# passcod/zarc

Hardware: AMD Instinct MI355X
Metric: uncompressed GiB/s (pack) at zstd -3 (higher is better)
Workload: dtype u8; 1 GPU; zarc pack 10000 x 1048576 B synthetic entries per GPU, zstd level 3, checksum on (BASELINE configs[1]); entries_per_gpu=10000, entries_total=10000, entry_bytes=1048576, level=3, kinds=text/records/lz/random round-robin

## Files before the change

### zarc_amd/csrc/zge_entropy.hip

```cpp
#include "zarc_device.h"
#include "zarc_kernels.h"
#include "zge_seq_join.h"

namespace {

#ifdef ZARC_HIPEMU
#define ZGE_CLOCK() 0ull
#else
#define ZGE_CLOCK() ((unsigned long long)__builtin_readcyclecounter())
#endif
#define ENT_PROF(i) do { if (prof && lane == 0) { const unsigned long long now_ = ZGE_CLOCK(); atomicAdd(prof + (i), now_ - tprev); tprev = now_; } } while (0)

constexpr int HUF_MAXBITS = 11;
constexpr uint32_t MIN_HUF_LITERALS = 64;

__constant__ const int16_t E_LL_DEFAULT[36] = {4, 3, 2, 2, 2, 2, 2, 2, 2, 2, 2, 2, 2, 1, 1, 1, 2, 2,
                                               2, 2, 2, 2, 2, 2, 2, 3, 2, 1, 1, 1, 1, 1, -1, -1, -1, -1};
__constant__ const int16_t E_ML_DEFAULT[53] = {1, 4, 3, 2, 2, 2, 2, 2, 2, 1, 1, 1, 1, 1, 1, 1, 1, 1,
                                               1, 1, 1, 1, 1, 1, 1, 1, 1, 1, 1, 1, 1, 1, 1, 1, 1, 1,
                                               1, 1, 1, 1, 1, 1, 1, 1, 1, 1, -1, -1, -1, -1, -1, -1, -1};
__constant__ const int16_t E_OF_DEFAULT[29] = {1, 1, 1, 1, 1, 1, 2, 2, 2, 1, 1, 1, 1, 1, 1,
                                               1, 1, 1, 1, 1, 1, 1, 1, 1, -1, -1, -1, -1, -1};
__device__ __forceinline__ uint32_t ll_code(uint32_t ll)
{
// ... 155 lines not shown
            rank++;
        }
    }
    zd::wave_sync();
    for (int i0 = 0; i0 < T; i0 += 64) {
        const int i = i0 + lane;
        const bool act = i < T;
        const uint32_t sym = act ? (uint32_t)cellsym[i] : 64u;
        uint64_t same = zd::ballot(act);
#pragma unroll
        for (int b = 0; b < 6; b++) { const uint64_t m = zd::ballot((sym >> b) & 1u); same &= ((sym >> b) & 1u) ? m : ~m; }
        const uint32_t below = (uint32_t)__popcll(same & ((1ull << lane) - 1)), all = (uint32_t)__popcll(same);
        int base = 0;
        if (act) base = t.dfs[sym];
        zd::wave_lds_order();
        if (act) {
            t.state_tab[base + (int)below] = (uint16_t)(T + i);
            if (below + 1 == all) t.dfs[sym] = base + (int)all;
        }
        zd::wave_lds_order();
    }
    zd::wave_sync();
    if (lane < nsym) {
        const int n = n_l, total = (int)start_all;
        if (n == 0) { t.dnb[lane] = ((al + 1) << 16) - T; t.dfs[lane] = 0; }
        else if (n == -1 || n == 1) { t.dnb[lane] = (al << 16) - T; t.dfs[lane] = total - 1; }
        else {
            const int max_bits_out = al - zd::hb32((uint32_t)(n - 1));
            t.dnb[lane] = (max_bits_out << 16) - (n << max_bits_out);
            t.dfs[lane] = total - n;
        }
    }
    t.al = al;
    zd::wave_sync();
}
__device__ __forceinline__ uint32_t fse_init_state(const FseCtab &t, int s)
{
    const int nb = (t.dnb[s] + (1 << 15)) >> 16;
    const int value = (nb << 16) - t.dnb[s];
    return t.state_tab[(value >> nb) + t.dfs[s]];
}
__device__ __forceinline__ uint32_t fse_step(const FseCtab &t, uint32_t state, int s, uint32_t *bits)
{
    const int nb = (int)((state + (uint32_t)t.dnb[s]) >> 16);
    *bits = (state & ((1u << nb) - 1)) | ((uint32_t)nb << 16);
    return t.state_tab[(int)(state >> nb) + t.dfs[s]];
}
__device__ uint32_t log2_fp8(uint32_t x)
{
    const int h = zd::hb32(x);
    const uint32_t frac = h >= 8 ? (x >> (h - 8)) - 256 : (x << (8 - h)) - 256;
    return (uint32_t)h * 256 + frac;
}
__device__ void fse_normalize(const uint32_t *count, int nsym, uint32_t total, int al, int16_t *norm)
{
    const int T = 1 << al;
    int sum = 0;
    for (int s = 0; s < nsym; s++) {
        if (count[s] == 0) { norm[s] = 0; continue; }
        uint64_t v = ((uint64_t)count[s] * (uint64_t)T + total / 2) / total;
        if (v < 1) v = 1;
        norm[s] = (int16_t)v;
        sum += (int)v;
    }
    while (sum != T) {
        int best = -1;
        for (int s = 0; s < nsym; s++) if (norm[s] > 0 && (best < 0 || norm[s] > norm[best])) best = s;
        if (sum > T) {
            int take = sum - T;
            const int room = norm[best] - 1;
            if (take > room) take = room;
            if (take <= 0) break;
            norm[best] = (int16_t)(norm[best] - take);
            sum -= take;
        } else {
            norm[best] = (int16_t)(norm[best] + (T - sum));
            sum = T;
        }
    }
}
__device__ uint32_t fse_write_desc(uint8_t *dst, uint32_t cap, const int16_t *norm, int nsym, int al)
{
    BitW b;
    b.init(dst, cap);
    int remaining = (1 << al) + 1, threshold = 1 << al, nb = al + 1, s = 0;
    b.add((uint32_t)(al - 5), 4);
    while (remaining > 1 && s < nsym) {
        const int count = norm[s++], max = 2 * threshold - 1 - remaining;
        int val = count + 1;
        remaining -= count < 0 ? -count : count;
        if (val >= threshold) val += max;
        if (val < max) b.add((uint32_t)val, nb - 1); else b.add((uint32_t)val, nb);
        if (count == 0) {
            int run = 0;
            while (s + run < nsym && norm[s + run] == 0) run++;
            s += run;
            while (run >= 3) { b.add(3, 2); run -= 3; }
            b.add((uint32_t)run, 2);
        }
        while (remaining < threshold) { nb--; threshold >>= 1; }
    }
    b.flush_partial();
    return b.overflow ? 0 : b.pos;
}
__device__ uint64_t dist_cost(const uint32_t *count, const int16_t *norm, int nsym, int al)
{
    uint64_t c = 0;
    for (int s = 0; s < nsym; s++) {
        if (!count[s]) continue;
        if (norm[s] == 0) return ~0ull;
        const uint32_t n = norm[s] < 0 ? 1u : (uint32_t)norm[s];
        c += (uint64_t)count[s] * ((uint32_t)al * 256 - log2_fp8(n));
    }
    return c;
}
__device__ void choose_table(EntLds &L, int which, const uint32_t *count, int maxsym, uint32_t nseq, const int16_t *def, int def_n,
                             int def_al, int max_al)
{
    int distinct = 0, last = 0;
    for (int s = 0; s <= maxsym; s++) if (count[s]) { distinct++; last = s; }
    int16_t *norm = L.s.norm[which];
    L.ctrl[X_COST_L + which] = 0;
    if (distinct == 1) { L.ctrl[X_MODE_L + which] = 1; L.ctrl[X_RLE_L + which] = last; L.ctrl[X_DL_L + which] = 0; return; }
    uint64_t cost_def = ~0ull;
    if (last < def_n) {
        for (int s = 0; s < def_n; s++) norm[s] = def[s];
        cost_def = dist_cost(count, norm, def_n, def_al);
    }
    int al = zd::hb32(nseq > 1 ? nseq - 1 : 1) - 2;
    if (al > max_al) al = max_al;
    if (al < 5) al = 5;
    while ((1 << al) < distinct) al++;
    const int nsym = last + 1;
    fse_normalize(count, nsym, nseq, al, norm);
    const uint32_t dl = fse_write_desc(L.s.desc[which], 80, norm, nsym, al);
    const uint64_t cost_dyn = dl ? dist_cost(count, norm, nsym, al) + (uint64_t)dl * 8 * 256 : ~0ull;
    if (cost_def <= cost_dyn) {
        for (int s = 0; s < def_n; s++) norm[s] = def[s];
        L.ctrl[X_MODE_L + which] = 0; L.ctrl[X_NSYM_L + which] = def_n; L.ctrl[X_AL_L + which] = def_al; L.ctrl[X_DL_L + which] = 0;
        L.ctrl[X_COST_L + which] = (int)(uint32_t)cost_def;
    } else {
        L.ctrl[X_MODE_L + which] = 2; L.ctrl[X_NSYM_L + which] = nsym; L.ctrl[X_AL_L + which] = al; L.ctrl[X_DL_L + which] = (int)dl;
        L.ctrl[X_COST_L + which] = (int)(uint32_t)cost_dyn;
    }
}

__device__ int huf_build_lengths(EntLds &L, int lane)
{
    uint32_t present = 0;
    uint32_t *const keys = &L.h.w[256];
    {
        const uint64_t lt = (1ull << lane) - 1;
#pragma unroll
        for (int r = 0; r < 4; r++) {
            const int s = r * 64 + lane;
            const uint32_t c = L.h.count[s];
            L.h.len8[s] = 0;
            const uint64_t m = zd::ballot(c != 0);
            if (c) keys[present + (uint32_t)__popcll(m & lt)] = (c << 8) | (uint32_t)s;
            present += (uint32_t)__popcll(m);
        }
    }
    zd::wave_sync();
    for (uint32_t i = (uint32_t)lane; i < present; i += 64) {
        const uint32_t k = keys[i];
        uint32_t rank = 0;
        for (uint32_t t = 0; t < present; t++) rank += keys[t] < k ? 1u : 0u;
        L.h.order[rank] = (uint16_t)(k & 0xFF);
    }
    zd::wave_sync();
    const int n = (int)present;
    if (n < 2) { if (n == 1 && lane == 0) L.h.len8[L.h.order[0]] = 1; zd::wave_sync(); return n; }
    for (int i = lane; i < n; i += 64) L.h.w[i] = L.h.count[L.h.order[i]];
    zd::wave_sync();
    if (lane == 0) {
        int leaf = 0, inode = n, next = n;
        while (next < 2 * n - 1) {
            int a, b;
            if (leaf < n && (inode >= next || L.h.w[leaf] <= L.h.w[inode])) a = leaf++; else a = inode++;
            if (leaf < n && (inode >= next || L.h.w[leaf] <= L.h.w[inode])) b = leaf++; else b = inode++;
            L.h.w[next] = L.h.w[a] + L.h.w[b];
            L.h.parent[a] = (uint16_t)next;
            L.h.parent[b] = (uint16_t)next;
            next++;
        }
    }
    zd::wave_sync();
    int *const num = (int *)&L.h.w[0];
    {
        uint32_t dep[4];
#pragma unroll
        for (int r = 0; r < 4; r++) {
            const int i = r * 64 + lane;
            dep[r] = 0;
            if (i < n) { int j = i; uint32_t d = 0; while (j != 2 * n - 2) { j = L.h.parent[j]; d++; } dep[r] = d > 63 ? 63 : d; }
        }
        zd::wave_sync();
// ... 17 lines not shown
    {
        uint32_t cum[HUF_MAXBITS + 1];
        uint32_t c = 0;
#pragma unroll
        for (int k = 1; k <= HUF_MAXBITS; k++) { c += (uint32_t)num[k]; cum[k] = c; }
#pragma unroll
        for (int r = 0; r < 4; r++) {
            const int j = r * 64 + lane;
            if (j < n) {
                const uint32_t t = (uint32_t)(n - 1 - j);
                uint32_t k = 1;
#pragma unroll
                for (int q = 1; q < HUF_MAXBITS; q++) k += cum[q] <= t ? 1u : 0u;
                L.h.len8[L.h.order[j]] = (uint8_t)k;
            }
        }
    }
    zd::wave_sync();
    return n;
}

__device__ void huf_assign_codes(EntLds &L, int lane)
{
    uint32_t len[4], idx[4];
    uint32_t maxlen = 0, last = 0;
#pragma unroll
    for (int r = 0; r < 4; r++) { len[r] = L.h.len8[r * 64 + lane]; idx[r] = 0; if (len[r] > maxlen) maxlen = len[r]; if (len[r]) last = (uint32_t)(r * 64 + lane); }
    maxlen = zd::uniform(zd::wave_max(maxlen));
    last = zd::uniform(zd::wave_max(last));
    const uint64_t lt = (1ull << lane) - 1;
    uint32_t *const rank_start = &L.h.w[64];
    uint32_t pos = 0;
    for (uint32_t w = 1; w <= maxlen; w++) {
        const uint32_t lv = maxlen + 1 - w;
        uint32_t cnt = 0;
#pragma unroll
        for (int r = 0; r < 4; r++) {
            const uint64_t m = zd::ballot(len[r] == lv);
            if (len[r] == lv) idx[r] = cnt + (uint32_t)__popcll(m & lt);
            cnt += (uint32_t)__popcll(m);
        }
        if (lane == 0) rank_start[w] = pos;
        pos += cnt << (w - 1);
    }
    zd::wave_sync();
#pragma unroll
    for (int r = 0; r < 4; r++) {
        uint32_t code = 0;
        if (len[r]) { const uint32_t w = maxlen + 1 - len[r]; code = ((rank_start[w] >> (w - 1)) + idx[r]) | (len[r] << 11); }
        L.code[r * 64 + lane] = (uint16_t)code;
    }
    if (lane == 0) { L.ctrl[X_MAXBITS] = (int)maxlen; L.ctrl[X_NSYM_LAST] = (int)last; }
    zd::wave_sync();
}

__device__ uint32_t huf_write_desc(EntLds &L)
{
    const int n = L.ctrl[X_NSYM_LAST];
    if (n > 1) {
        int nsym = 0, distinct = 0, al = 6;
        uint32_t maxc = 0;
        for (int s = 0; s < 13; s++) if (L.h.cw[s]) { nsym = s + 1; distinct++; if (L.h.cw[s] > maxc) maxc = L.h.cw[s]; }
        if (distinct > 1 && maxc > 1) {
            { int lim = zd::hb32((uint32_t)(n - 1)) - 2; if (lim < al) al = lim; if (al < 5) al = 5; }
            while ((1 << al) < distinct) al++;
            fse_normalize(L.h.cw, nsym, (uint32_t)n, al, L.h.wnorm);
            const uint32_t hdr = fse_write_desc(L.h.tmp, 192, L.h.wnorm, nsym, al);
            if (hdr) {
                FseCtab ct = {L.h.st_w, L.h.dnb_w, L.h.dfs_w, 0};
                fse_build_ctab(ct, L.h.wnorm, nsym, al, L.cellsym);
                BitW b;
                b.init(L.h.tmp + hdr, 192 - hdr);
                uint32_t s1, s2, bits;
                int ip = n;
                if (n & 1) {
                    s1 = fse_init_state(ct, L.h.wt[--ip]);
                    s2 = fse_init_state(ct, L.h.wt[--ip]);
                    s1 = fse_step(ct, s1, L.h.wt[--ip], &bits); b.add(bits & 0xFFFF, (int)(bits >> 16));
                } else {
                    s2 = fse_init_state(ct, L.h.wt[--ip]);
                    s1 = fse_init_state(ct, L.h.wt[--ip]);
                }
                while (ip > 0) {
                    s2 = fse_step(ct, s2, L.h.wt[--ip], &bits); b.add(bits & 0xFFFF, (int)(bits >> 16));
                    s1 = fse_step(ct, s1, L.h.wt[--ip], &bits); b.add(bits & 0xFFFF, (int)(bits >> 16));
                }
                b.add(s2, al);
                b.add(s1, al);
                const uint32_t body = b.close();
                if (!b.overflow && hdr + body < 128 && (n > 128 || hdr + body < (uint32_t)(n + 1) / 2)) {
                    L.h.hdesc[0] = (uint8_t)(hdr + body);
                    for (uint32_t i = 0; i < hdr + body; i++) L.h.hdesc[1 + i] = L.h.tmp[i];
                    return 1 + hdr + body;
                }
            }
        }
    }
    if (n > 128) return 0;
    L.h.hdesc[0] = (uint8_t)(127 + n);
    for (int i = 0; i < n; i += 2) L.h.hdesc[1 + i / 2] = (uint8_t)((L.h.wt[i] << 4) | (i + 1 < n ? L.h.wt[i + 1] : 0));
    return (uint32_t)(1 + (n + 1) / 2);
}

struct WavePacker {
    uint32_t *stage;
    uint8_t *dst;
    uint32_t pos;
    uint32_t carry;
    uint32_t cap;
    bool overflow;
    __device__ void begin(uint32_t *st, uint8_t *d, uint32_t c, int lane)
    {
        stage = st; dst = d; pos = 0; carry = 0; cap = c; overflow = false;
        for (int i = lane; i < 224; i += 64) stage[i] = 0;
        zd::wave_sync();
    }
    __device__ void put(uint64_t lo, uint32_t hi, uint32_t nbits, int lane)
    {
        const uint32_t incl = zd::wave_scan_incl(nbits);
        const uint32_t total = zd::readlane(incl, 63);
        const uint32_t at = carry + incl - nbits;
        if (nbits) {
            const uint32_t w = at >> 5, sh = at & 31;
            const uint32_t v0 = (uint32_t)lo, v1 = (uint32_t)(lo >> 32), v2 = hi;
            const uint32_t o0 = v0 << sh;
            const uint32_t o1 = sh ? (v1 << sh) | (v0 >> (32 - sh)) : v1;
            const uint32_t o2 = sh ? (v2 << sh) | (v1 >> (32 - sh)) : v2;
            const uint32_t o3 = sh ? (v2 >> (32 - sh)) : 0u;
            if (o0) atomicOr(&stage[w], o0);
            if (o1) atomicOr(&stage[w + 1], o1);
            if (o2) atomicOr(&stage[w + 2], o2);
            if (o3) atomicOr(&stage[w + 3], o3);
        }
        zd::wave_sync();
        const uint32_t bits = carry + total, full = bits >> 3;
        const uint8_t *sb = (const uint8_t *)stage;
        if (pos + full + 1 > cap) overflow = true;
        if (!overflow) {
            const uint32_t fw = full >> 2;
            for (uint32_t i = (uint32_t)lane; i < fw; i += 64) { const uint32_t w = stage[i]; __builtin_memcpy(dst + pos + 4 * i, &w, 4); }
            if ((uint32_t)lane < (full & 3)) dst[pos + 4 * fw + (uint32_t)lane] = sb[4 * fw + (uint32_t)lane];
        }
        const uint32_t keep = (bits & 7) ? (uint32_t)sb[full] : 0u;
        zd::wave_sync();
        const uint32_t words = (bits + 31) / 32 + 1;
        for (uint32_t i = (uint32_t)lane; i < words; i += 64) stage[i] = i == 0 ? keep : 0u;
        zd::wave_sync();
        pos += full;
        carry = bits & 7;
    }
    __device__ uint32_t finish(int lane)
    {
        put(1, 0, lane == 0 ? 1u : 0u, lane);
        if (carry) {
            if (lane == 0 && !overflow) dst[pos] = (uint8_t)stage[0];
            pos += 1;
            carry = 0;
        }
        return pos;
    }
};

template <int PHASE, bool SPLIT>
__device__ __forceinline__ void zge_entropy_body(EntLds &L, uint32_t n_blocks, uint32_t slot_bytes, ZgeBlock *__restrict__ blocks, uint64_t *__restrict__ seq_scratch,
                                                 const uint8_t *__restrict__ lit_scratch, uint8_t *__restrict__ out_scratch,
                                                 unsigned long long *__restrict__ prof , ZgePlan *__restrict__ plans,
                                                 uint32_t *__restrict__ err , const ZgePiece *__restrict__ pieces,
                                                 const uint32_t bi)
{
    const int lane = zd::lane_id();
    unsigned long long tprev = ZGE_CLOCK();
    if (bi >= n_blocks) return;
    ZgeBlock *rec = blocks + bi;
    ZgePlan *const plan = PHASE ? plans + bi : nullptr;
    if (PHASE == 2 && !plan->active) return;
    if (rec->type == 1 || (SPLIT && rec->type == ZGE_PIECE_UNUSED)) { if (PHASE == 1 && lane == 0) plan->active = 0; return; }
    const uint32_t nlit = rec->nlit, src_len = rec->src_len;
    uint32_t nseq = PHASE == 2 ? plan->nseq : rec->nseq;
    const uint32_t slot_i = SPLIT ? bi / ZGE_SPLIT_K : bi;
    const uint32_t seq_first = SPLIT ? pieces[bi].seq_first : 0u, lit_first = SPLIT ? pieces[bi].lit_first : 0u;
    uint64_t *seq = seq_scratch + (uint64_t)slot_i * zge_seq_stride(slot_bytes) + seq_first;
    const uint8_t *lit = lit_scratch + (uint64_t)slot_i * zge_lit_stride(slot_bytes) + lit_first;
    uint8_t *out = out_scratch + (uint64_t)slot_i * zge_out_stride(slot_bytes) + (SPLIT ? pieces[bi].out_off : 0u);
    const uint32_t out_cap = SPLIT ? pieces[bi].out_cap : (uint32_t)zge_out_stride(slot_bytes);
    bool fail = false;
    constexpr bool STATES = PHASE == 2 && !SPLIT;
    const bool given = STATES && plan->states != 0;
    const uint32_t *const swords = (const uint32_t *)(lit_scratch + (uint64_t)slot_i * zge_lit_stride(slot_bytes));

    uint32_t lsz = PHASE == 2 ? plan->lsz : 0u;
    if (PHASE != 2) {
        const uint32_t n = nlit;
        const uint32_t raw_hdr = n < 32 ? 1u : (n < 4096 ? 2u : 3u);
        for (int i = lane; i < 256; i += 64) L.h.count[i] = 0;
        zd::wave_sync();
        {
            const uint32_t n4 = n / 4;
            const uint32_t *l4 = (const uint32_t *)lit;
            for (uint32_t i0 = 0; i0 < n4; i0 += 256) {
                uint32_t wv[4];
#pragma unroll
                for (uint32_t k = 0; k < 4; k++) { const uint32_t i = i0 + 64 * k + (uint32_t)lane; wv[k] = i < n4 ? l4[i] : 0u; }
#pragma unroll
                for (uint32_t k = 0; k < 4; k++) {
                    if (i0 + 64 * k + (uint32_t)lane >= n4) continue;
                    const uint32_t w = wv[k];
                    atomicAdd(&L.h.count[w & 0xFF], 1u); atomicAdd(&L.h.count[(w >> 8) & 0xFF], 1u);
                    atomicAdd(&L.h.count[(w >> 16) & 0xFF], 1u); atomicAdd(&L.h.count[w >> 24], 1u);
                }
            }
            for (uint32_t i = n4 * 4 + (uint32_t)lane; i < n; i += 64) atomicAdd(&L.h.count[lit[i]], 1u);
        }
        zd::wave_sync();
        ENT_PROF(0);
        uint32_t distinct = 0;
#pragma unroll
        for (int r = 0; r < 4; r++) distinct += (uint32_t)__popcll(zd::ballot(L.h.count[r * 64 + lane] != 0));
        uint32_t largest = 0;
#pragma unroll
        for (int r = 0; r < 4; r++) { const uint32_t c = L.h.count[r * 64 + lane]; largest = c > largest ? c : largest; }
        largest = zd::uniform(zd::wave_max(largest));
        const bool flat = largest <= (n >> 7) + 4;
        int kind = 0;
        if (n >= 2 && distinct == 1) kind = 1;
        else if (n >= MIN_HUF_LITERALS && distinct >= 2 && !flat) {
            huf_build_lengths(L, lane);
            huf_assign_codes(L, lane);
            uint32_t est_bits = 0;
            {
                const int max_bits = L.ctrl[X_MAXBITS], nlast = L.ctrl[X_NSYM_LAST];
                if (lane < 16) L.h.cw[lane] = 0;
                zd::wave_sync();
#pragma unroll
                for (int r = 0; r < 4; r++) {
                    const int sym = r * 64 + lane;
                    const uint32_t l = L.h.len8[sym];
                    const uint32_t wgt = l ? (uint32_t)(max_bits + 1 - (int)l) : 0u;
                    L.h.wt[sym] = (uint8_t)wgt;
                    if (sym < nlast) atomicAdd(&L.h.cw[wgt], 1u);
                    est_bits += L.h.count[sym] * l;
                }
                est_bits = zd::uniform(zd::wave_sum(est_bits));
            }
            zd::wave_sync();
            if (lane == 0) {
                const uint32_t dlen = huf_write_desc(L);
                const uint64_t est = dlen + ((uint64_t)est_bits + 7) / 8 + (n >= 256 ? 10 : 1);
                L.ctrl[X_DLEN] = (dlen && est + 3 < n) ? (int)dlen : 0;
            }
            zd::wave_sync();
            ENT_PROF(1);
            const uint32_t dlen = (uint32_t)L.ctrl[X_DLEN];
            zd::wave_sync();
            if (dlen) {
                const bool single = n < 256;
                const uint32_t hdr = single ? 3u : (n < 1024 ? 3u : (n < 16384 ? 4u : 5u));
                uint8_t *body = out + hdr;
                for (uint32_t i = (uint32_t)lane; i < dlen; i += 64) body[i] = L.h.hdesc[i];
                uint32_t pos = dlen, ssz[4] = {0, 0, 0, 0};
                const uint32_t nstreams = single ? 1u : 4u, per = single ? n : (n + 3) / 4, jt = pos;
                if (!single) pos += 6;
                WavePacker pk;
#pragma unroll
                for (uint32_t k = 0; k < 4; k++) {
                    if (k >= nstreams) break;
                    const uint32_t beg = k * per, cnt = single ? n : (k < 3 ? per : n - 3 * per);
                    pk.begin(L.stage, body + pos, out_cap - hdr - pos, lane);
                    for (uint32_t j0 = 0; j0 < cnt; j0 += 512) {
                        const uint32_t j = j0 + 8 * (uint32_t)lane;
                        uint64_t ca = 0, cb = 0;
                        uint32_t na = 0, nb_ = 0;
                        if (j + 8 <= cnt) {
                            uint64_t w;
                            __builtin_memcpy(&w, lit + beg + cnt - 8 - j, 8);
#pragma unroll
                            for (uint32_t q = 0; q < 4; q++) { const uint32_t e = L.code[(w >> (8 * (7 - q))) & 0xFF]; ca |= (uint64_t)(e & 0x7FF) << na; na += e >> 11; }
#pragma unroll
                            for (uint32_t q = 4; q < 8; q++) { const uint32_t e = L.code[(w >> (8 * (7 - q))) & 0xFF]; cb |= (uint64_t)(e & 0x7FF) << nb_; nb_ += e >> 11; }
                        } else if (j < cnt) {
                            for (uint32_t q = 0; q < 4 && j + q < cnt; q++) { const uint32_t e = L.code[lit[beg + cnt - 1 - j - q]]; ca |= (uint64_t)(e & 0x7FF) << na; na += e >> 11; }
                            for (uint32_t q = 4; q < 8 && j + q < cnt; q++) { const uint32_t e = L.code[lit[beg + cnt - 1 - j - q]]; cb |= (uint64_t)(e & 0x7FF) << nb_; nb_ += e >> 11; }
                        }
                        const uint64_t lo = ca | (na < 64 ? cb << na : 0ull);
                        const uint32_t hi = na ? (uint32_t)(cb >> (64 - na)) : 0u;
                        pk.put(lo, hi, na + nb_, lane);
                    }
                    ssz[k] = pk.finish(lane);
                    if (pk.overflow) fail = true;
                    pos += ssz[k];
                }
                if (!single) {
                    if (lane == 0) for (int k = 0; k < 3; k++) { body[jt + 2 * k] = (uint8_t)ssz[k]; body[jt + 2 * k + 1] = (uint8_t)(ssz[k] >> 8); }
                    if (ssz[0] > 65535 || ssz[1] > 65535 || ssz[2] > 65535) fail = true;
                }
                const uint32_t comp = pos;
                if (!fail && comp + hdr < n + raw_hdr) {
                    uint64_t v;
                    if (hdr == 3) v = 2u | ((single ? 0u : 1u) << 2) | ((uint64_t)n << 4) | ((uint64_t)comp << 14);
                    else if (hdr == 4) v = 2u | (2u << 2) | ((uint64_t)n << 4) | ((uint64_t)comp << 18);
                    else v = 2u | (3u << 2) | ((uint64_t)n << 4) | ((uint64_t)comp << 22);
                    if (lane == 0) for (uint32_t i = 0; i < hdr; i++) out[i] = (uint8_t)(v >> (8 * i));
                    lsz = hdr + comp;
                    kind = 2;
                }
            }
        }
// ... 44 lines not shown
            const uint32_t src1 = zd::shfl(a, nk1 ? 63 - __clzll((long long)nk1) : 0);
            const uint32_t r1_after = nk1 ? src1 : r1;
            uint32_t bb = zd::shfl_up1(r1_after);
            if (lane == 0) bb = r1;
            const bool keep2 = !valid || (z ? o == bb : (o == a || o == bb));
            const uint64_t nk2 = zd::ballot(!keep2) & upto;
            const uint32_t src2 = zd::shfl(bb, nk2 ? 63 - __clzll((long long)nk2) : 0);
            const uint32_t r2_after = nk2 ? src2 : r2;
            uint32_t c = zd::shfl_up1(r2_after);
            if (lane == 0) c = r2;
            uint32_t ofv;
            if (!z) ofv = o == a ? 1u : (o == bb ? 2u : (o == c ? 3u : o + 3));
            else ofv = o == bb ? 1u : (o == c ? 2u : ((a > 1 && o == a - 1) ? 3u : o + 3));
            if (valid) seq[base + (uint32_t)lane] = zge_pack_seq(ll, ml, ofv);
            r0 = zd::readlane(o, cnt - 1);
            r1 = zd::readlane(r1_after, cnt - 1);
            r2 = zd::readlane(r2_after, cnt - 1);
        }
        zd::wave_sync_global();
    }
    ENT_PROF(3);

    uint32_t ssz = 0;
    if (!fail) {
        uint8_t *so = out + lsz;
        const uint32_t scap = out_cap - lsz;
        uint32_t pos = 0;
        if (lane == 0) {
            if (nseq < 128) so[0] = (uint8_t)nseq;
            else if (nseq < 0x7F00) { so[0] = (uint8_t)((nseq >> 8) + 128); so[1] = (uint8_t)nseq; }
            else { so[0] = 255; so[1] = (uint8_t)(nseq - 0x7F00); so[2] = (uint8_t)((nseq - 0x7F00) >> 8); }
        }
        pos = nseq < 128 ? 1u : (nseq < 0x7F00 ? 2u : 3u);
        if (nseq == 0) ssz = pos;
        else {
          if (PHASE != 2) {
            for (int i = lane; i < 36; i += 64) L.s.cl[i] = 0;
            for (int i = lane; i < 32; i += 64) L.s.co[i] = 0;
            for (int i = lane; i < 53; i += 64) L.s.cm[i] = 0;
            zd::wave_sync();
            for (uint32_t i0 = 0; i0 < nseq; i0 += 256) {
                uint64_t sv[4];
#pragma unroll
                for (uint32_t k = 0; k < 4; k++) { const uint32_t i = i0 + 64 * k + (uint32_t)lane; sv[k] = i < nseq ? seq[i] : 0; }
#pragma unroll
                for (uint32_t k = 0; k < 4; k++) {
                    if (i0 + 64 * k + (uint32_t)lane >= nseq) continue;
                    atomicAdd(&L.s.cl[ll_code(zge_seq_ll(sv[k]))], 1u);
                    atomicAdd(&L.s.cm[ml_code(zge_seq_ml(sv[k]))], 1u);
                    atomicAdd(&L.s.co[zd::hb32(zge_seq_ofv(sv[k]))], 1u);
                }
            }
            zd::wave_sync();
            if (lane < 3) {
                const int which = lane;
                const uint32_t *cnt = which == 0 ? L.s.cl : (which == 1 ? L.s.co : L.s.cm);
                const int16_t *def = which == 0 ? E_LL_DEFAULT : (which == 1 ? E_OF_DEFAULT : E_ML_DEFAULT);
                choose_table(L, which, cnt, which == 0 ? 35 : (which == 1 ? 31 : 52), nseq, def, which == 0 ? 36 : (which == 1 ? 29 : 53),
                             which == 1 ? 5 : 6, which == 1 ? 8 : 9);
            }
            zd::wave_sync();
          }
          if (PHASE == 1) {
#pragma unroll
            for (int which = 0; which < 3; which++) {
                ZgePlanTable *pt = &plan->t[which];
                const uint32_t *cnt = which == 0 ? L.s.cl : (which == 1 ? L.s.co : L.s.cm);
                const int nc = which == 0 ? 36 : (which == 1 ? 32 : 53);
                pt->count[lane] = lane < nc ? cnt[lane] : 0u;
                pt->norm[lane] = L.s.norm[which][lane];
                pt->desc[lane] = L.s.desc[which][lane];
                if (lane < 16) pt->desc[64 + lane] = L.s.desc[which][64 + lane];
                if (lane == 0) {
                    pt->cost = (uint32_t)L.ctrl[X_COST_L + which];
                    pt->mode = (uint8_t)L.ctrl[X_MODE_L + which]; pt->al = (uint8_t)L.ctrl[X_AL_L + which]; pt->nsym = (uint8_t)L.ctrl[X_NSYM_L + which];
                    pt->dl = (uint8_t)L.ctrl[X_DL_L + which]; pt->rle = (uint8_t)L.ctrl[X_RLE_L + which];
                }
            }
            {
                uint32_t xb = 0;
                if (lane < 36) xb += L.s.cl[lane] * ll_code_bits((uint32_t)lane);
                if (lane < 53) xb += L.s.cm[lane] * ml_code_bits((uint32_t)lane);
                if (lane < 32) xb += L.s.co[lane] * (uint32_t)lane;
                xb = zd::wave_sum(xb);
                if (lane == 0) { plan->active = 1; plan->nseq = nseq; plan->lsz = lsz; plan->extra_bits = xb; plan->guaranteed = 0; if (!SPLIT) plan->states = 0; }
            }
            return;
          }
          if (PHASE == 2) {
#pragma unroll
            for (int which = 0; which < 3; which++) {
                const ZgePlanTable *pt = &plan->t[which];
                L.s.norm[which][lane] = pt->norm[lane];
                L.s.desc[which][lane] = pt->desc[lane];
                if (lane < 16) L.s.desc[which][64 + lane] = pt->desc[64 + lane];
                if (lane == 0) {
                    L.ctrl[X_MODE_L + which] = pt->mode; L.ctrl[X_AL_L + which] = pt->al; L.ctrl[X_NSYM_L + which] = pt->nsym;
                    L.ctrl[X_DL_L + which] = pt->dl; L.ctrl[X_RLE_L + which] = pt->rle;
                }
            }
            zd::wave_sync();
          }
#pragma unroll
            for (int which = 0; which < 3; which++) {
                FseCtab tt = which == 0 ? FseCtab{L.s.st + ST_LL, L.s.dnb_ll, L.s.dfs_ll, 0}
                                        : (which == 1 ? FseCtab{L.s.st + ST_OF, L.s.dnb_of, L.s.dfs_of, 0} : FseCtab{L.s.st + ST_ML, L.s.dnb_ml, L.s.dfs_ml, 0});
                uint8_t *cells = (uint8_t *)L.s.pre;
                if (STATES && given) {
                    if (L.ctrl[X_MODE_L + which] != 1 && lane < L.ctrl[X_NSYM_L + which]) tt.dnb[lane] = fse_sym_dnb(L.s.norm[which][lane], L.ctrl[X_AL_L + which]);
                } else if (L.ctrl[X_MODE_L + which] != 1) fse_build_ctab_wave(tt, L.s.norm[which], L.ctrl[X_NSYM_L + which], L.ctrl[X_AL_L + which], cells, lane);
#ifdef ZGE_DEBUG_FSE
                if (L.ctrl[X_MODE_L + which] != 1 && lane == 0) {
// ... 163 lines not shown
    ZGE_SPLIT_LOOP zge_entropy_body<0, true>(L, n_blocks * ZGE_SPLIT_K, slot_bytes, blocks, seq_scratch, lit_scratch, out_scratch, prof, nullptr, nullptr, pieces, blockIdx.x * ZGE_SPLIT_K + k);
}
__global__ void __launch_bounds__(64, 5) zarc_zge_entropy_p1_split(ZGE_ENTROPY_ARGS, ZgePlan *__restrict__ plans, const ZgePiece *__restrict__ pieces)
{
    __shared__ EntLds L;
    ZGE_SPLIT_LOOP zge_entropy_body<1, true>(L, n_blocks * ZGE_SPLIT_K, slot_bytes, blocks, seq_scratch, lit_scratch, out_scratch, prof, plans, nullptr, pieces, blockIdx.x * ZGE_SPLIT_K + k);
    const uint32_t idle = (uint32_t)zd::lane_id();
    if (idle >= np && idle < ZGE_SPLIT_K) plans[(uint64_t)blockIdx.x * ZGE_SPLIT_K + idle].active = 0;
}
__global__ void __launch_bounds__(64, 5) zarc_zge_entropy_p2_split(ZGE_ENTROPY_ARGS, ZgePlan *__restrict__ plans, uint32_t *__restrict__ err,
                                                                   const ZgePiece *__restrict__ pieces)
{
    __shared__ EntLds L;
    ZGE_SPLIT_LOOP zge_entropy_body<2, true>(L, n_blocks * ZGE_SPLIT_K, slot_bytes, blocks, seq_scratch, lit_scratch, out_scratch, prof, plans, err, pieces, blockIdx.x * ZGE_SPLIT_K + k);
}
#undef ZGE_ENTROPY_ARGS
#undef ZGE_SPLIT_LOOP

namespace {
template <bool SPLIT>
__device__ __forceinline__ void zge_plan_body(int16_t (*gnorm)[64], uint8_t (*gdesc)[80], uint32_t *gdl, uint32_t n_blocks, const ZgeBlock *__restrict__ blocks,
                                              ZgePlan *__restrict__ plans, const uint32_t *__restrict__ group_start, const ZgeBlock *__restrict__ pblocks)
{
    const int lane = zd::lane_id();
    const uint32_t bi = group_start[blockIdx.x];
    if (bi >= n_blocks) return;
    const uint32_t frame = blocks[bi].frame, index0 = blocks[bi].index;
    if (index0 % ZGE_TABLE_GROUP) return;
    uint32_t nb = 1;
    while (nb < ZGE_TABLE_GROUP && bi + nb < n_blocks && blocks[bi + nb].frame == frame && blocks[bi + nb].index == index0 + nb) nb++;
    if (!SPLIT && nb < 2) return;
    const ZgeBlock *const recs = SPLIT ? pblocks + (uint64_t)bi * ZGE_SPLIT_K : blocks + bi;
    plans += SPLIT ? (uint64_t)bi * ZGE_SPLIT_K : (uint64_t)bi;
    if (SPLIT) nb *= ZGE_SPLIT_K;
    bool use_group[3] = {false, false, false};
    uint32_t g_al[3] = {0, 0, 0}, g_nsym[3] = {0, 0, 0};
#pragma unroll
    for (int t = 0; t < 3; t++) {
        const int max_al = t == 1 ? 8 : 9;
        uint32_t sum = 0, total = 0, cost_own = 0, np = 0;
        for (uint32_t b = 0; b < nb; b++) {
            const ZgePlan *p = plans + b;
            if (!p->active || p->t[t].mode == 1) continue;
            sum += p->t[t].count[lane];
            total += p->nseq; cost_own += p->t[t].cost; np++;
        }
        if (np < 2) continue;
        const uint64_t present = zd::ballot(sum != 0);
        const int distinct = (int)__popcll(present), last = 63 - (int)__clzll((long long)present);
        int al = zd::hb32(total > 1 ? total - 1 : 1) - 2;
        if (al > max_al) al = max_al;
        if (al < 5) al = 5;
        while ((1 << al) < distinct) al++;
        const uint32_t T = 1u << al;
        uint32_t v = 0;
        if (sum) { v = (sum * T + total / 2) / total; if (v < 1) v = 1; }
        uint32_t vs = zd::uniform(zd::wave_sum(v));
        while (vs != T) {
            const uint32_t key = v ? (v << 6) | (uint32_t)(63 - lane) : 0u;
            const uint32_t best = 63u - (zd::uniform(zd::wave_max(key)) & 63u);
            const uint32_t bv = zd::readlane(v, best);
            if (vs > T) {
                uint32_t take = vs - T;
                const uint32_t room = bv - 1;
                if (take > room) take = room;
                if (take == 0) break;
                if ((uint32_t)lane == best) v -= take;
                vs -= take;
            } else {
                if ((uint32_t)lane == best) v += T - vs;
                vs = T;
            }
        }
        gnorm[t][lane] = (int16_t)v;
        zd::wave_sync();
        if (lane == 0) gdl[t] = fse_write_desc(gdesc[t], 80, gnorm[t], last + 1, al);
        zd::wave_sync();
        const uint32_t dl = gdl[t];
        if (!dl) continue;
        const uint32_t cost_group = zd::uniform(zd::wave_sum(sum ? sum * ((uint32_t)al * 256 - log2_fp8(v)) : 0u)) + dl * 8 * 256;
        use_group[t] = cost_group <= cost_own + (cost_own >> 6);
        g_al[t] = (uint32_t)al; g_nsym[t] = (uint32_t)(last + 1);
    }
    if (!use_group[0] && !use_group[1] && !use_group[2]) return;
    bool have[3] = {false, false, false};
    bool entry[3] = {false, false, false}, prev_cut = false;
    for (uint32_t b = 0; b < nb; b++) {
        ZgePlan *p = plans + b;
        if (SPLIT && b % ZGE_SPLIT_K == 0) {
#pragma unroll
            for (int t = 0; t < 3; t++) { if (prev_cut) have[t] = have[t] && entry[t]; entry[t] = have[t]; }
            prev_cut = recs[b].pad > 1;
        }
        if (!p->active) continue;
        uint32_t ub_bits = 1 + p->extra_bits, hdrs = 0;
        bool grp[3];
#pragma unroll
        for (int t = 0; t < 3; t++) {
            ZgePlanTable *pt = &p->t[t];
            uint32_t mode = pt->mode, al = pt->al, dl = pt->dl;
            int n_l = pt->norm[lane];
            grp[t] = mode != 1 && use_group[t];
            if (grp[t]) {
                mode = have[t] ? 3u : 2u; al = g_al[t]; dl = mode == 2 ? gdl[t] : 0u; n_l = gnorm[t][lane];
                pt->norm[lane] = (int16_t)n_l;
                if (mode == 2) { pt->desc[lane] = gdesc[t][lane]; if (lane < 16) pt->desc[64 + lane] = gdesc[t][64 + lane]; }
                if (lane == 0) { pt->mode = (uint8_t)mode; pt->al = (uint8_t)al; pt->nsym = (uint8_t)g_nsym[t]; pt->dl = (uint8_t)dl; }
            }
            if (mode != 1) {
                const uint32_t cnt = pt->count[lane];
                const uint32_t mb = (n_l == -1 || n_l == 1) ? al : (n_l > 1 ? al - (uint32_t)zd::hb32((uint32_t)(n_l - 1)) : 0u);
                ub_bits += zd::uniform(zd::wave_sum(cnt * mb)) + al;
            }
            hdrs += mode == 1 ? 1u : dl;
        }
        const uint32_t nseq = p->nseq;
        const uint32_t ub = p->lsz + (nseq < 128 ? 1u : (nseq < 0x7F00 ? 2u : 3u)) + 1 + (ub_bits + 7) / 8 + hdrs;
        const bool guaranteed = ub < recs[b].src_len;
        if (lane == 0) p->guaranteed = guaranteed ? 1u : 0u;
#pragma unroll
        for (int t = 0; t < 3; t++) have[t] = grp[t] && guaranteed;
    }
}
}

__global__ void __launch_bounds__(64) zarc_zge_plan(uint32_t n_blocks, const ZgeBlock *__restrict__ blocks, ZgePlan *__restrict__ plans,
                                                    const uint32_t *__restrict__ group_start )
{
    __shared__ int16_t gnorm[3][64];
    __shared__ uint8_t gdesc[3][80];
    __shared__ uint32_t gdl[3];
    zge_plan_body<false>(gnorm, gdesc, gdl, n_blocks, blocks, plans, group_start, nullptr);
}
// ... 154 lines not shown
```

Baseline: 45.70 GiB/s.

## Parallelize FSE table choice and Huffman weight descriptor across the wave

Replaces the serial lane-0 (or lanes 0-2) FSE normalization, cost evaluation, NCount header writing and Huffman-weight FSE encoding with wave-wide versions. These use ballots, scans and a WavePacker to emit bitfields in parallel. The Huffman weight stream is encoded with two interleaved states on lanes 0 and 1 and then packed by all lanes. The three table choices now run sequentially per wave instead of on three lanes at once. The intent is to remove long single-lane serial sections in the entropy stage, at the cost of more wave-wide reductions and some subtle bit-packing logic that must exactly match the serial output.

Result: no change. 46.03 GiB/s, median of 6 (+0.7%).

```diff
diff --git a/zarc_amd/csrc/zge_entropy.hip b/zarc_amd/csrc/zge_entropy.hip
--- a/zarc_amd/csrc/zge_entropy.hip
+++ b/zarc_amd/csrc/zge_entropy.hip
@@ -231,33 +231,6 @@
     const uint32_t frac = h >= 8 ? (x >> (h - 8)) - 256 : (x << (8 - h)) - 256;
     return (uint32_t)h * 256 + frac;
 }
-__device__ void fse_normalize(const uint32_t *count, int nsym, uint32_t total, int al, int16_t *norm)
-{
-    const int T = 1 << al;
-    int sum = 0;
-    for (int s = 0; s < nsym; s++) {
-        if (count[s] == 0) { norm[s] = 0; continue; }
-        uint64_t v = ((uint64_t)count[s] * (uint64_t)T + total / 2) / total;
-        if (v < 1) v = 1;
-        norm[s] = (int16_t)v;
-        sum += (int)v;
-    }
-    while (sum != T) {
-        int best = -1;
-        for (int s = 0; s < nsym; s++) if (norm[s] > 0 && (best < 0 || norm[s] > norm[best])) best = s;
-        if (sum > T) {
-            int take = sum - T;
-            const int room = norm[best] - 1;
-            if (take > room) take = room;
-            if (take <= 0) break;
-            norm[best] = (int16_t)(norm[best] - take);
-            sum -= take;
-        } else {
-            norm[best] = (int16_t)(norm[best] + (T - sum));
-            sum = T;
-        }
-    }
-}
 __device__ uint32_t fse_write_desc(uint8_t *dst, uint32_t cap, const int16_t *norm, int nsym, int al)
 {
     BitW b;
@@ -282,46 +255,33 @@
     b.flush_partial();
     return b.overflow ? 0 : b.pos;
 }
-__device__ uint64_t dist_cost(const uint32_t *count, const int16_t *norm, int nsym, int al)
-{
-    uint64_t c = 0;
-    for (int s = 0; s < nsym; s++) {
-        if (!count[s]) continue;
-        if (norm[s] == 0) return ~0ull;
-        const uint32_t n = norm[s] < 0 ? 1u : (uint32_t)norm[s];
-        c += (uint64_t)count[s] * ((uint32_t)al * 256 - log2_fp8(n));
-    }
-    return c;
-}
-__device__ void choose_table(EntLds &L, int which, const uint32_t *count, int maxsym, uint32_t nseq, const int16_t *def, int def_n,
-                             int def_al, int max_al)
-{
-    int distinct = 0, last = 0;
-    for (int s = 0; s <= maxsym; s++) if (count[s]) { distinct++; last = s; }
-    int16_t *norm = L.s.norm[which];
-    L.ctrl[X_COST_L + which] = 0;
-    if (distinct == 1) { L.ctrl[X_MODE_L + which] = 1; L.ctrl[X_RLE_L + which] = last; L.ctrl[X_DL_L + which] = 0; return; }
-    uint64_t cost_def = ~0ull;
-    if (last < def_n) {
-        for (int s = 0; s < def_n; s++) norm[s] = def[s];
-        cost_def = dist_cost(count, norm, def_n, def_al);
-    }
-    int al = zd::hb32(nseq > 1 ? nseq - 1 : 1) - 2;
-    if (al > max_al) al = max_al;
-    if (al < 5) al = 5;
-    while ((1 << al) < distinct) al++;
-    const int nsym = last + 1;
-    fse_normalize(count, nsym, nseq, al, norm);
-    const uint32_t dl = fse_write_desc(L.s.desc[which], 80, norm, nsym, al);
-    const uint64_t cost_dyn = dl ? dist_cost(count, norm, nsym, al) + (uint64_t)dl * 8 * 256 : ~0ull;
-    if (cost_def <= cost_dyn) {
-        for (int s = 0; s < def_n; s++) norm[s] = def[s];
-        L.ctrl[X_MODE_L + which] = 0; L.ctrl[X_NSYM_L + which] = def_n; L.ctrl[X_AL_L + which] = def_al; L.ctrl[X_DL_L + which] = 0;
-        L.ctrl[X_COST_L + which] = (int)(uint32_t)cost_def;
-    } else {
-        L.ctrl[X_MODE_L + which] = 2; L.ctrl[X_NSYM_L + which] = nsym; L.ctrl[X_AL_L + which] = al; L.ctrl[X_DL_L + which] = (int)dl;
-        L.ctrl[X_COST_L + which] = (int)(uint32_t)cost_dyn;
-    }
+__device__ __forceinline__ uint32_t fse_normalize_wave(uint32_t cnt, uint32_t total, int al, int lane)
+{
+    const uint32_t T = 1u << al;
+    uint32_t v = 0;
+    if (cnt) { v = (cnt * T + total / 2) / total; if (v < 1) v = 1; }
+    uint32_t vs = zd::readlane(zd::wave_scan_incl(v), 63);
+    while (vs != T) {
+        const uint32_t key = v ? (v << 6) | (uint32_t)(63 - lane) : 0u;
+        const uint32_t best = 63u - (zd::uniform(zd::wave_max(key)) & 63u);
+        const uint32_t bv = zd::readlane(v, best);
+        if (vs > T) {
+            uint32_t take = vs - T;
+            const uint32_t room = bv - 1;
+            if (take > room) take = room;
+            if (take == 0) break;
+            if ((uint32_t)lane == best) v -= take;
+            vs -= take;
+        } else {
+            if ((uint32_t)lane == best) v += T - vs;
+            vs = T;
+        }
+    }
+    return v;
+}
+__device__ __forceinline__ uint32_t fse_cost_wave(uint32_t cnt, uint32_t n, int al)
+{
+    return zd::readlane(zd::wave_scan_incl(cnt ? cnt * ((uint32_t)al * 256 - log2_fp8(n)) : 0u), 63);
 }
 
 __device__ int huf_build_lengths(EntLds &L, int lane)
@@ -445,54 +405,6 @@
     }
     if (lane == 0) { L.ctrl[X_MAXBITS] = (int)maxlen; L.ctrl[X_NSYM_LAST] = (int)last; }
     zd::wave_sync();
-}
-
-__device__ uint32_t huf_write_desc(EntLds &L)
-{
-    const int n = L.ctrl[X_NSYM_LAST];
-    if (n > 1) {
-        int nsym = 0, distinct = 0, al = 6;
-        uint32_t maxc = 0;
-        for (int s = 0; s < 13; s++) if (L.h.cw[s]) { nsym = s + 1; distinct++; if (L.h.cw[s] > maxc) maxc = L.h.cw[s]; }
-        if (distinct > 1 && maxc > 1) {
-            { int lim = zd::hb32((uint32_t)(n - 1)) - 2; if (lim < al) al = lim; if (al < 5) al = 5; }
-            while ((1 << al) < distinct) al++;
-            fse_normalize(L.h.cw, nsym, (uint32_t)n, al, L.h.wnorm);
-            const uint32_t hdr = fse_write_desc(L.h.tmp, 192, L.h.wnorm, nsym, al);
-            if (hdr) {
-                FseCtab ct = {L.h.st_w, L.h.dnb_w, L.h.dfs_w, 0};
-                fse_build_ctab(ct, L.h.wnorm, nsym, al, L.cellsym);
-                BitW b;
-                b.init(L.h.tmp + hdr, 192 - hdr);
-                uint32_t s1, s2, bits;
-                int ip = n;
-                if (n & 1) {
-                    s1 = fse_init_state(ct, L.h.wt[--ip]);
-                    s2 = fse_init_state(ct, L.h.wt[--ip]);
-                    s1 = fse_step(ct, s1, L.h.wt[--ip], &bits); b.add(bits & 0xFFFF, (int)(bits >> 16));
-                } else {
-                    s2 = fse_init_state(ct, L.h.wt[--ip]);
-                    s1 = fse_init_state(ct, L.h.wt[--ip]);
-                }
-                while (ip > 0) {
-                    s2 = fse_step(ct, s2, L.h.wt[--ip], &bits); b.add(bits & 0xFFFF, (int)(bits >> 16));
-                    s1 = fse_step(ct, s1, L.h.wt[--ip], &bits); b.add(bits & 0xFFFF, (int)(bits >> 16));
-                }
-                b.add(s2, al);
-                b.add(s1, al);
-                const uint32_t body = b.close();
-                if (!b.overflow && hdr + body < 128 && (n > 128 || hdr + body < (uint32_t)(n + 1) / 2)) {
-                    L.h.hdesc[0] = (uint8_t)(hdr + body);
-                    for (uint32_t i = 0; i < hdr + body; i++) L.h.hdesc[1 + i] = L.h.tmp[i];
-                    return 1 + hdr + body;
-                }
-            }
-        }
-    }
-    if (n > 128) return 0;
-    L.h.hdesc[0] = (uint8_t)(127 + n);
-    for (int i = 0; i < n; i += 2) L.h.hdesc[1 + i / 2] = (uint8_t)((L.h.wt[i] << 4) | (i + 1 < n ? L.h.wt[i + 1] : 0));
-    return (uint32_t)(1 + (n + 1) / 2);
 }
 
 struct WavePacker {
@@ -552,7 +464,140 @@
         }
         return pos;
     }
+    __device__ uint32_t finish_plain(int lane)
+    {
+        if (carry) {
+            if (lane == 0 && !overflow) dst[pos] = (uint8_t)stage[0];
+            pos += 1;
+            carry = 0;
+        }
+        return pos;
+    }
 };
+
+__device__ __forceinline__ uint32_t fse_write_desc_wave(uint32_t *stage, uint8_t *dst, uint32_t cap, int n, int nsym, int al, int lane)
+{
+    const bool in = lane < nsym;
+    const uint32_t a = in ? (uint32_t)(n < 0 ? -n : n) : 0u;
+    const int remaining = (1 << al) + 1 - (int)(zd::wave_scan_incl(a) - a);
+    const uint64_t zm = zd::ballot(in && n == 0);
+    const bool follower = lane > 0 && ((zm >> lane) & 1) && ((zm >> (lane - 1)) & 1);
+    uint64_t field = 0;
+    uint32_t bits = 0;
+    if (in && remaining > 1 && !follower) {
+        const int hb = zd::hb32((uint32_t)remaining), threshold = 1 << hb, max = 2 * threshold - 1 - remaining;
+        int val = n + 1;
+        if (val >= threshold) val += max;
+        bits = (uint32_t)(val < max ? hb : hb + 1);
+        field = (uint32_t)val & ((1u << bits) - 1);
+        if (n == 0) {
+            const uint64_t rest = lane < 63 ? zm >> (lane + 1) : 0ull;
+            const uint32_t run = (uint32_t)zd::ctz64(~rest), q = run / 3, r = run - 3 * q;
+            field |= ((((uint64_t)1 << (2 * q)) - 1) | ((uint64_t)r << (2 * q))) << bits;
+            bits += 2 * (q + 1);
+        }
+    }
+    if (lane == 0) { field = (field << 4) | (uint32_t)(al - 5); bits += 4; }
+    WavePacker pk;
+    pk.begin(stage, dst, cap, lane);
+    pk.put(field, 0, bits, lane);
+    const uint32_t len = pk.finish_plain(lane);
+    return pk.overflow ? 0u : len;
+}
+
+template <int WHICH>
+__device__ __forceinline__ void choose_table_wave(EntLds &L, uint32_t c, uint32_t nseq, int lane)
+{
+    constexpr int def_n = WHICH == 0 ? 36 : (WHICH == 1 ? 29 : 53), def_al = WHICH == 1 ? 5 : 6, max_al = WHICH == 1 ? 8 : 9;
+    const int16_t *const def = WHICH == 0 ? E_LL_DEFAULT : (WHICH == 1 ? E_OF_DEFAULT : E_ML_DEFAULT);
+    const uint64_t present = zd::ballot(c != 0);
+    const int distinct = (int)__popcll(present), last = 63 - (int)__clzll((long long)present);
+    if (distinct == 1) {
+        if (lane == 0) { L.ctrl[X_COST_L + WHICH] = 0; L.ctrl[X_MODE_L + WHICH] = 1; L.ctrl[X_RLE_L + WHICH] = last; L.ctrl[X_DL_L + WHICH] = 0; }
+        return;
+    }
+    const int d = lane < def_n ? (int)def[lane] : 0;
+    uint64_t cost_def = ~0ull;
+    if (last < def_n) cost_def = fse_cost_wave(c, d <= 0 ? 1u : (uint32_t)d, def_al);
+    int al = zd::hb32(nseq > 1 ? nseq - 1 : 1) - 2;
+    if (al > max_al) al = max_al;
+    if (al < 5) al = 5;
+    while ((1 << al) < distinct) al++;
+    const uint32_t v = fse_normalize_wave(c, nseq, al, lane);
+    const uint32_t dl = fse_write_desc_wave(L.stage, L.s.desc[WHICH], 80, (int)v, last + 1, al, lane);
+    const uint64_t cost_dyn = dl ? (uint64_t)fse_cost_wave(c, v ? v : 1u, al) + (uint64_t)dl * 8 * 256 : ~0ull;
+    if (cost_def <= cost_dyn) {
+        L.s.norm[WHICH][lane] = (int16_t)d;
+        if (lane == 0) {
+            L.ctrl[X_MODE_L + WHICH] = 0; L.ctrl[X_NSYM_L + WHICH] = def_n; L.ctrl[X_AL_L + WHICH] = def_al; L.ctrl[X_DL_L + WHICH] = 0;
+            L.ctrl[X_COST_L + WHICH] = (int)(uint32_t)cost_def;
+        }
+    } else {
+        L.s.norm[WHICH][lane] = (int16_t)v;
+        if (lane == 0) {
+            L.ctrl[X_MODE_L + WHICH] = 2; L.ctrl[X_NSYM_L + WHICH] = last + 1; L.ctrl[X_AL_L + WHICH] = al; L.ctrl[X_DL_L + WHICH] = (int)dl;
+            L.ctrl[X_COST_L + WHICH] = (int)(uint32_t)cost_dyn;
+        }
+    }
+}
+
+__device__ __forceinline__ uint32_t huf_write_desc_wave(EntLds &L, int lane)
+{
+    const int n = (int)zd::uniform((uint32_t)L.ctrl[X_NSYM_LAST]);
+    if (n > 1) {
+        const uint32_t c = lane < 13 ? L.h.cw[lane] : 0u;
+        const uint64_t present = zd::ballot(c != 0);
+        const int distinct = (int)__popcll(present), nsym = 64 - (int)__clzll((long long)present);
+        const uint32_t maxc = zd::uniform(zd::wave_max(c));
+        if (distinct > 1 && maxc > 1) {
+            int al = 6;
+            { int lim = zd::hb32((uint32_t)(n - 1)) - 2; if (lim < al) al = lim; if (al < 5) al = 5; }
+            while ((1 << al) < distinct) al++;
+            const uint32_t v = fse_normalize_wave(c, (uint32_t)n, al, lane);
+            if (lane < 16) L.h.wnorm[lane] = (int16_t)v;
+            const uint32_t hdr = fse_write_desc_wave(L.stage, L.h.tmp, 192, (int)v, nsym, al, lane);
+            zd::wave_sync();
+            if (hdr) {
+                FseCtab ct = {L.h.st_w, L.h.dnb_w, L.h.dfs_w, 0};
+                fse_build_ctab_wave(ct, L.h.wnorm, nsym, al, L.cellsym, lane);
+                uint32_t *const eb = &L.h.w[0];
+                uint32_t state = 0;
+                if (lane < 2) {
+                    int i = n - 1 - lane;
+                    state = fse_init_state(ct, L.h.wt[i]);
+                    for (i -= 2; i >= 0; i -= 2) { uint32_t bits; state = fse_step(ct, state, L.h.wt[i], &bits); eb[i] = bits; }
+                }
+                zd::wave_sync();
+                const uint32_t c0 = zd::readlane(state, 0), c1 = zd::readlane(state, 1), mask = (1u << al) - 1;
+                const uint32_t fin = (n & 1) ? (c1 & mask) | ((c0 & mask) << al) : (c0 & mask) | ((c1 & mask) << al);
+                uint64_t lo = 0;
+                uint32_t nb = 0;
+#pragma unroll
+                for (int q = 0; q < 4; q++) {
+                    const int k = 4 * lane + q;
+                    if (k + 2 < n) { const uint32_t e = eb[n - 3 - k]; lo |= (uint64_t)(e & 0xFFFF) << nb; nb += e >> 16; }
+                    else if (k + 2 == n) { lo |= (uint64_t)fin << nb; nb += 2 * (uint32_t)al; }
+                }
+                WavePacker pk;
+                pk.begin(L.stage, L.h.tmp + hdr, 192 - hdr, lane);
+                pk.put(lo, 0, nb, lane);
+                const uint32_t body = pk.finish(lane);
+                zd::wave_sync();
+                if (!pk.overflow && hdr + body < 128 && (n > 128 || hdr + body < (uint32_t)(n + 1) / 2)) {
+                    if (lane == 0) L.h.hdesc[0] = (uint8_t)(hdr + body);
+                    for (uint32_t i = (uint32_t)lane; i < hdr + body; i += 64) L.h.hdesc[1 + i] = L.h.tmp[i];
+                    zd::wave_sync();
+                    return 1 + hdr + body;
+                }
+            }
+        }
+    }
+    if (n > 128) return 0;
+    if (lane == 0) L.h.hdesc[0] = (uint8_t)(127 + n);
+    if (2 * lane < n) L.h.hdesc[1 + lane] = (uint8_t)((L.h.wt[2 * lane] << 4) | (2 * lane + 1 < n ? L.h.wt[2 * lane + 1] : 0));
+    zd::wave_sync();
+    return (uint32_t)(1 + (n + 1) / 2);
+}
 
 template <int PHASE, bool SPLIT>
 __device__ __forceinline__ void zge_entropy_body(EntLds &L, uint32_t n_blocks, uint32_t slot_bytes, ZgeBlock *__restrict__ blocks, uint64_t *__restrict__ seq_scratch,
@@ -636,15 +681,9 @@
                 est_bits = zd::uniform(zd::wave_sum(est_bits));
             }
             zd::wave_sync();
-            if (lane == 0) {
-                const uint32_t dlen = huf_write_desc(L);
-                const uint64_t est = dlen + ((uint64_t)est_bits + 7) / 8 + (n >= 256 ? 10 : 1);
-                L.ctrl[X_DLEN] = (dlen && est + 3 < n) ? (int)dlen : 0;
-            }
-            zd::wave_sync();
+            uint32_t dlen = huf_write_desc_wave(L, lane);
+            if (!(dlen && dlen + ((uint64_t)est_bits + 7) / 8 + (n >= 256 ? 10 : 1) + 3 < n)) dlen = 0;
             ENT_PROF(1);
-            const uint32_t dlen = (uint32_t)L.ctrl[X_DLEN];
-            zd::wave_sync();
             if (dlen) {
                 const bool single = n < 256;
                 const uint32_t hdr = single ? 3u : (n < 1024 ? 3u : (n < 16384 ? 4u : 5u));
@@ -795,12 +834,10 @@
                 }
             }
             zd::wave_sync();
-            if (lane < 3) {
-                const int which = lane;
-                const uint32_t *cnt = which == 0 ? L.s.cl : (which == 1 ? L.s.co : L.s.cm);
-                const int16_t *def = which == 0 ? E_LL_DEFAULT : (which == 1 ? E_OF_DEFAULT : E_ML_DEFAULT);
-                choose_table(L, which, cnt, which == 0 ? 35 : (which == 1 ? 31 : 52), nseq, def, which == 0 ? 36 : (which == 1 ? 29 : 53),
-                             which == 1 ? 5 : 6, which == 1 ? 8 : 9);
+            {
+                choose_table_wave<0>(L, lane < 36 ? L.s.cl[lane] : 0u, nseq, lane);
+                choose_table_wave<1>(L, lane < 32 ? L.s.co[lane] : 0u, nseq, lane);
+                choose_table_wave<2>(L, lane < 53 ? L.s.cm[lane] : 0u, nseq, lane);
             }
             zd::wave_sync();
           }
@@ -1070,33 +1107,14 @@
         if (al > max_al) al = max_al;
         if (al < 5) al = 5;
         while ((1 << al) < distinct) al++;
-        const uint32_t T = 1u << al;
-        uint32_t v = 0;
-        if (sum) { v = (sum * T + total / 2) / total; if (v < 1) v = 1; }
-        uint32_t vs = zd::uniform(zd::wave_sum(v));
-        while (vs != T) {
-            const uint32_t key = v ? (v << 6) | (uint32_t)(63 - lane) : 0u;
-            const uint32_t best = 63u - (zd::uniform(zd::wave_max(key)) & 63u);
-            const uint32_t bv = zd::readlane(v, best);
-            if (vs > T) {
-                uint32_t take = vs - T;
-                const uint32_t room = bv - 1;
-                if (take > room) take = room;
-                if (take == 0) break;
-                if ((uint32_t)lane == best) v -= take;
-                vs -= take;
-            } else {
-                if ((uint32_t)lane == best) v += T - vs;
-                vs = T;
-            }
-        }
+        const uint32_t v = fse_normalize_wave(sum, total, al, lane);
         gnorm[t][lane] = (int16_t)v;
         zd::wave_sync();
         if (lane == 0) gdl[t] = fse_write_desc(gdesc[t], 80, gnorm[t], last + 1, al);
         zd::wave_sync();
         const uint32_t dl = gdl[t];
         if (!dl) continue;
-        const uint32_t cost_group = zd::uniform(zd::wave_sum(sum ? sum * ((uint32_t)al * 256 - log2_fp8(v)) : 0u)) + dl * 8 * 256;
+        const uint32_t cost_group = fse_cost_wave(sum, v, al) + dl * 8 * 256;
         use_group[t] = cost_group <= cost_own + (cost_own >> 6);
         g_al[t] = (uint32_t)al; g_nsym[t] = (uint32_t)(last + 1);
     }
```
